# kthohr/mcmc

Measured on AMD Instinct MI355X. Metric: leapfrog-steps/sec (chains*dims*steps/s), HMC d=128 correlated Gaussian, 65536 chains, higher is better.
Workload: dtype f64

## Files before the change

include/mi_mcmc_engine/nuts_memo_core.hpp:

```cpp
#pragma once

#ifndef MI_MEMO_WALK_CAP
#define MI_MEMO_WALK_CAP 8
#endif

#ifndef MI_MEMO_RNG_ILP
#define MI_MEMO_RNG_ILP 1
#endif

#ifndef MI_MEMO_WALK_V2
#define MI_MEMO_WALK_V2 1
#endif
#ifndef MI_MEMO_APF
#define MI_MEMO_APF 0
#endif

#include "hmc_dense.hpp"

namespace mi {
namespace memo {

enum : int { NS_NEED_DRAW = 0, NS_TREE = 1, NS_DONE = 2,
             NS_INIT = 3, NS_SEARCH = 4,
             NS_WAIT = 5 };
enum : uint32_t { PQ_EMPTY = 0xffffffffu, PQ_GONE = 0xfffffffeu };
template <class T> __device__ __forceinline__ T coh_ld(const T* p) { return __hip_atomic_load(p, __ATOMIC_RELAXED, __HIP_MEMORY_SCOPE_AGENT); }
template <class T> __device__ __forceinline__ void coh_st(T* p, T v) { __hip_atomic_store(p, v, __ATOMIC_RELAXED, __HIP_MEMORY_SCOPE_AGENT); }
enum : int {
    MV_PREV = 0, MV_WPREV = 1, MV_MNTM = 2, MV_TPOS_T = 3, MV_TPOS_P = 4, MV_TNEG_T = 5, MV_TNEG_P = 6,
    MV_MNTM2 = 7, MV_PREVB = 8, MV_WPREVB = 9,
    MV_PT0 = 10,
    MEMO_MAXPTS = 46,
    MEMO_NVEC = MV_PT0 + 3 * MEMO_MAXPTS,
    MEMO_MAX_DEPTH = 10
};
enum : int {
    R_LA = 0,
    R_SC = 11,
    R_NF = 15,
    R_DA = 16,
    R_OKB = 19,
    R_LP = 31,
    R_CH = 42,
    R_CT = 49,
    R_END = 52
};
constexpr size_t lds_bytes() { return (size_t)R_END * 512 + 10 * 48 * 2; }

__host__ __device__ constexpr size_t memo_wave_bytes(int NS) { return (size_t)MEMO_NVEC * NS * 512 + (size_t)(MEMO_MAXPTS + 1) * 64 * 16; }

__device__ __forceinline__ uint32_t memo_npt(uint32_t i)
{
    return 1u + (uint32_t)__builtin_popcount(i) + (uint32_t)__builtin_popcount(i & 0x2AAu) + 2u * (uint32_t)__builtin_popcount(i & 0xCCu)
         + 4u * (uint32_t)__builtin_popcount(i & 0xF0u) + 8u * (uint32_t)__builtin_popcount(i & 0x300u);
}
__host__ __device__ inline bool memo_pair_used(int l, int n1, int j)
{
    const int m = n1 - 1;
    for (int t = 0; t <= j - l; ++t) {
        const int lo = t * (l + 1) + t * (t - 1) / 2, hi = t * j - t * (t - 1) / 2;
        if (m >= lo && m <= hi) return true;
    }
    return false;
}

template <int NT, class POL, class PRM>
__device__ __forceinline__ void nuts_memo_run(const PRM& prm, POL& pol, char* const lds_rows, uint16_t* const lds_pm)
{
    constexpr int NS = 4 * NT;
    for (int i = threadIdx.x; i < 10 * 48; i += blockDim.x) {
        const int j = i / 48, m = i % 48;
        uint32_t bits = 0;
        for (int l = 1; l <= j; ++l)
            if (m - l >= 1 && memo_pair_used(l, m - l, j)) bits |= 1u << l;
        lds_pm[i] = (uint16_t)bits;
    }
    __syncthreads();

    const int lane = threadIdx.x & 63, wave = threadIdx.x >> 6;
    const int j4 = lane >> 4;
    const int cw = wave * 16 + (lane & 15);
    const uint32_t d = prm.d;
    const uint64_t C = prm.C;
    const uint32_t nw = blockDim.x >> 6;
    const uint64_t n_slots = (uint64_t)gridDim.x * (16u * nw);
    uint64_t cl = ((uint64_t)blockIdx.x * nw + wave) * 16 + (lane & 15);
    bool exhausted = prm.next_chain == nullptr;
    uint32_t n_pieces = 1u, piece_len = 0xffffffffu;
    if constexpr (POL::SPLIT) { if (prm.n_pieces > 1u && prm.next_chain != nullptr) { n_pieces = prm.n_pieces; piece_len = prm.piece_len; } }
    const uint64_t n_items = C * (uint64_t)n_pieces;
    bool piece_done = false;

    typedef double __attribute__((address_space(3)))* lds_dptr;
    typedef unsigned long long __attribute__((address_space(3)))* lds_uptr;
    typedef char __attribute__((address_space(3)))* lds_bptr;
    uint32_t lrow = (uint32_t)(uintptr_t)(lds_bptr)lds_rows + (uint32_t)cw * 8u;
#define MI_RD(r) (*(lds_dptr)(uintptr_t)(lrow + (uint32_t)(r) * 512u))
#define MI_RU(r) (*(lds_uptr)(uintptr_t)(lrow + (uint32_t)(r) * 512u))
#define la_(l) MI_RD(R_LA + (l))
#define lp_(l) MI_RU(R_LP + (l))
#define okb_(r) MI_RU(R_OKB + (r))
#define nf_() MI_RD(R_NF)
    const int wave_u = __builtin_amdgcn_readfirstlane(wave);
    char* const ws_wave_u = reinterpret_cast<char*>(__builtin_assume_aligned(prm.ws, 256)) + ((size_t)blockIdx.x * nw + wave_u) * memo_wave_bytes(NS);
    uint32_t lane_b = (uint32_t)(lane & 15) * (uint32_t)(NS * 32) + (uint32_t)j4 * 16u;
    uint32_t lane_sc = (uint32_t)MEMO_NVEC * (uint32_t)(NS * 512) + (uint32_t)lane * 16u;
    auto wsp = [&](int v, int s) -> double* {
        return reinterpret_cast<double*>(ws_wave_u + ((uint32_t)v * (uint32_t)(NS * 512) + lane_b + (uint32_t)(s >> 1) * 64u));
    };
    auto scp = [&](uint32_t n) -> double2* { return reinterpret_cast<double2*>(ws_wave_u + (lane_sc + n * 1024u)); };
    auto ld_row = [&](int v, int s0, auto& dst) __attribute__((always_inline)) {
        constexpr int N = (int)(sizeof(dst) / sizeof(double));
        static_assert(N % 2 == 0, "rows move in pairs of slices");
#pragma unroll
        for (int k = 0; k < N; k += 2) {
            const double2 t = *reinterpret_cast<const double2*>(wsp(v, s0 + k));
            dst[k] = t.x; dst[k + 1] = t.y;
        }
    };
    auto st_row = [&](int v, int s0, const auto& src) __attribute__((always_inline)) {
        constexpr int N = (int)(sizeof(src) / sizeof(double));
        static_assert(N % 2 == 0, "rows move in pairs of slices");
#pragma unroll
        for (int k = 0; k < N; k += 2) *reinterpret_cast<double2*>(wsp(v, s0 + k)) = double2{src[k], src[k + 1]};
    };
#ifndef MI_MEMO_NT
#define MI_MEMO_NT 1
#endif
    [[maybe_unused]] auto st_row_nt = [&](int v, int s0, const auto& src) __attribute__((always_inline)) {
// ... 350 lines not shown
            if (gen) { next_K_() = kq / 2.0; next_lu_() = lu; mom_ready = true; }
            }
            const bool p = state == NS_NEED_DRAW;
            roll_state(p);
            if (max_depth > 0) begin_doubling(p);
            else { end_draw(p, 0u); if (p) state = NS_NEED_DRAW; }
        }
        const bool run = state == NS_TREE, init = state == NS_INIT, srch = state == NS_SEARCH;
        MI_MPROF(0)
        if (__ballot(run || init || srch) == 0ull) continue;
#ifdef MI_NUTS_REG_PROF
        n_ticks++; n_active += (unsigned long long)__builtin_popcountll(__ballot(run)) / 4ull;
        pc[10] += (unsigned long long)__builtin_popcountll(__ballot(run && memo_npt(li) > npts)) / 4ull;
#endif

        if (__ballot(init) != 0ull) {
#pragma unroll 1
            for (int b = 0; b < NS / 2; ++b) {
                const bool in0 = 8u * b + j4 < d, in1 = 8u * b + 4 + j4 < d;
                const double* src = prm.theta + ((size_t)(in0 ? 8u * b + j4 : 0u) * C + cl);
                double t0 = 0.0, t1 = 0.0;
                if (init) {
                    if constexpr (POL::SPLIT) { t0 = coh_ld(src); t1 = coh_ld(src + (in1 ? (size_t)4 * C : 0)); }
                    else { t0 = src[0]; t1 = src[in1 ? (size_t)4 * C : 0]; }
                }
                bool raw = false;
                if constexpr (POL::SPLIT) raw = draw != 0u;
                if (init) st_pair(MV_PREV, 2 * b, in0 ? (raw ? t0 : pol.enter(t0, 8 * b + j4)) : 0.0, in1 ? (raw ? t1 : pol.enter(t1, 8 * b + 4 + j4)) : 0.0);
            }
            const bool any_fresh = __ballot(init && prm.draw0 == 0 && draw == 0u) != 0ull;
#pragma unroll 1
            for (int b = 0; b < NS / 2; ++b) {
                double pa = 0.0, pb_ = 0.0;
                if (any_fresh) {
                    double z0, z1;
                    rng_normal_pair(prm.seed, prm.chain0 + cl, 0u, (uint32_t)(4 * b + j4), STREAM_INIT, z0, z1);
                    pa = (8u * b + j4 < d) ? z0 : 0.0;
                    pb_ = (8u * b + 4 + j4 < d) ? z1 : 0.0;
                    pa = pol.msqrt_times(pa, 8 * b + j4); pb_ = pol.msqrt_times(pb_, 8 * b + 4 + j4);
                }
                if (init) st_pair(mv, 2 * b, pa, pb_);
            }
        }
        const bool newpt = run && memo_npt(li) > npts;
        {
            const bool need = (newpt && npts == 0u && !org_ok) || init;
            if (__ballot(need) != 0ull) {
                const int vt = pvec(pb), vw = init ? pvec(pb) : wvec(pb);
                if (need) { ld_row(vt, 0, th); ld_draw_mom(init, pm); ld_row(vw, 0, w); }
            }
        }
        if (newpt) org_ok = false;
        const uint32_t mpt = npts + 1u;
        uint32_t pmask = newpt ? ((uint32_t)lds_pm[jd * 48u + mpt] | ((mpt == 1u + jd) ? 1u : 0u)) : 0u;
        auto test_vecs = [&](int l, int& vt, int& vp, bool& pmom) __attribute__((always_inline)) {
            vt = MV_PT0 + 3 * ((int)mpt - l - 1); vp = vt + 1; pmom = false;
            if (l == 0) {
                const bool oinit = (vdir > 0) ? neg_init : pos_init;
                vt = oinit ? pvec(pb0) : ((vdir > 0) ? MV_TNEG_T : MV_TPOS_T);
                vp = oinit ? mv : ((vdir > 0) ? MV_TNEG_P : MV_TPOS_P);
                pmom = oinit;
            }
        };
        auto ld_test_p = [&](int vp, bool pmom, auto& dst) __attribute__((always_inline)) {
            if constexpr (POL::PRE_MOM) ld_ptr(pmom ? mom_lane_ptr(draw) : ws_lane_ptr(vp), dst);
            else ld_row(vp, 0, dst);
        };
        double dd[NS], Lp[NS];
#pragma unroll
        for (int s_ = 0; s_ < NS; ++s_) { dd[s_] = 0.0; Lp[s_] = 0.0; }
        if (srch) {
            if (!s_first) eps_() = eps_() * ((vdir == 1) ? 2.0 : 0.5);
            n_leap_() += 1ull; n_exec_() += 1ull;
        }
        const double e_tick = newpt ? esg_() : (srch ? eps_() : 0.0);
#if MI_MEMO_APF > 0 && MI_MEMO_WALK_CAP > 0
        double apf[MI_MEMO_WALK_CAP];
#pragma unroll
        for (int k = 0; k < MI_MEMO_WALK_CAP; ++k) apf[k] = 0.0;
        auto request_alphas = [&]() __attribute__((always_inline)) {
            if (__ballot(run) == 0ull) return;
            uint32_t i_ = li, n_ = memo_npt(li);
            const uint32_t np_ = newpt ? mpt : npts;
            bool ok_ = run;
#pragma unroll
            for (int k = 0; k < MI_MEMO_WALK_CAP; ++k) {
                const uint32_t t_ = (uint32_t)__builtin_ctz(~i_);
                const uint32_t nn_ = n_ + (t_ + 1u) - t_ * (t_ + 1u) / 2u;
                ok_ = ok_ && nn_ <= np_;
                if (ok_ && !(newpt && nn_ == mpt)) apf[k] = scp(nn_)->x;
                i_ = i_ + 1u; n_ = nn_;
            }
        };
#endif
#if MI_MEMO_APF == 2 && MI_MEMO_WALK_CAP > 0
        request_alphas();
#endif
        const bool act = newpt || srch;
        pol.kick(th, pm, w, e_tick, act);
        pol.drift(th, pm, e_tick, act);
        __builtin_amdgcn_sched_barrier(0);
        {
            const bool t1 = pmask != 0u;
            if (__ballot(t1) != 0ull) {
                const int l1 = t1 ? __builtin_ctz(pmask) : 1;
                int vq, vqp; bool pmom;
                test_vecs(l1, vq, vqp, pmom);
                if (t1) { ld_row(vq, 0, dd); ld_test_p(vqp, pmom, Lp); }
            }
        }
        MI_MPROF(1)
        double val = 0.0;
        pol.eval(th, w, val);
        pol.kick(th, pm, w, e_tick, act);
        double pU = pol.potential(th, w, val);
        const double pK = pol.kinetic(pm);
        MI_MPROF(2)
        if (__ballot(init) != 0ull) {
            if (init) {
                st_row(MV_PREV, 0, th); st_row(MV_WPREV, 0, w);
                prev_U_() = pU;
                if constexpr (POL::REPLAY) { if (!is_finite(pU)) nf_() = 1.0; }
                H0_() = (is_finite(pU) ? pU : INF) + pK;
                s_first = true;
            }
            const bool cont = prm.draw0 != 0 || draw != 0u;
            if (init && cont) eps_() = prm.step_out ? coh_ld(prm.step_out + cl) : 1.0;
            start_sampling(init && cont);
            if (init && !cont) state = NS_SEARCH;
        }
        if (!is_finite(pU)) pU = INF;
        if (__ballot(srch) != 0ull) {
            const double dHs = -(pU + pK) + H0_();
            note_nonfinite(srch && !is_finite(dHs));
            if (srch) { vdir = 2 * (dHs > log_half ? 1 : 0) - 1; s_first = false; }
            start_sampling(srch && !(dHs > neg_log2));
        }
        MI_MPROF(5)
        if (__ballot(run) == 0ull) continue;
        const double dH = -(pU + pK) + H0_();
        note_nonfinite(newpt && !is_finite(dH));
        const double ca_pt = det_exp((dH < 0.0) ? dH : 0.0);
        if (newpt) {
            const unsigned long long bit = 1ull << mpt;
            const double lu_ = log_u_();
            const bool cn_b = lu_ <= -pU - pK;
            const bool cs_b = lu_ < 1000.0 - pU - pK;
            okb_(0) = (okb_(0) & ~bit) | (cn_b ? bit : 0ull);
            okb_(11) = (okb_(11) & ~bit) | (cs_b ? bit : 0ull);
            n_exec_() += 1ull;
        }
#if MI_MEMO_APF == 1 && MI_MEMO_WALK_CAP > 0
        request_alphas();
#endif
        MI_MPROF(8)
        {
            bool first = true;
#pragma unroll 1
            while (__ballot(pmask != 0u) != 0ull) {
#ifdef MI_NUTS_REG_PROF
                n_pair_it++;
#endif
                const bool t = pmask != 0u;
                const int l = t ? __builtin_ctz(pmask) : 1;
                const int n1 = (int)mpt - l;
                if (!first) {
                    int vq, vqp; bool pmom;
                    test_vecs(l, vq, vqp, pmom);
#if MI_MEMO_NT == 3
                    if (t) { ld_ptr_nt(ws_lane_ptr(vq), dd); if constexpr (POL::PRE_MOM) ld_ptr_nt(pmom ? mom_lane_ptr(draw) : ws_lane_ptr(vqp), Lp); else ld_ptr_nt(ws_lane_ptr(vqp), Lp); }
#else
                    if (t) { ld_row(vq, 0, dd); ld_test_p(vqp, pmom, Lp); }
#endif
                }
                first = false;
                double q1 = 0.0, q2 = 0.0;
#pragma unroll
                for (int s_ = 0; s_ < NS; ++s_) {
                    dd[s_] = (vdir > 0) ? (th[s_] - dd[s_]) : (dd[s_] - th[s_]);
                    q1 = dfma(dd[s_], Lp[s_], q1);
                }
                __builtin_amdgcn_sched_barrier(0);
#pragma unroll
                for (int s_ = 0; s_ < NS; ++s_) q2 = dfma(dd[s_], pm[s_], q2);
                q1 = q1 + __shfl_xor(q1, 32); q1 = q1 + __shfl_xor(q1, 16);
                q2 = q2 + __shfl_xor(q2, 32); q2 = q2 + __shfl_xor(q2, 16);
                if (t) {
                    const unsigned long long bit = (l == 0) ? (1ull << 63) : (1ull << n1);
                    const bool ok = (q1 >= 0.0) && (q2 >= 0.0);
                    okb_(l) = (okb_(l) & ~bit) | (ok ? bit : 0ull);
                    pmask &= pmask - 1u;
                }
            }
        }
        const bool st_edge = newpt && mpt == 1u + jd;
        if (st_edge) { if (vdir > 0) pos_init = false; else neg_init = false; }
        if (newpt) npts = mpt;
        MI_MPROF(3)
        bool wl = run;
        bool at_fin = false, complete = false;
        uint32_t cn_i = 0, cna_i = 0, cref = 0;
        double ca = newpt ? ca_pt : ca_keep;
        double ca_nx = 0.0;
        uint32_t n_walked = 0;
        uint32_t n = memo_npt(li);
#if MI_MEMO_WALK_CAP > 0
        int walk_budget = MI_MEMO_WALK_CAP;
#endif
#pragma unroll 1
        while (__ballot(wl) != 0ull) {
#ifdef MI_NUTS_REG_PROF
            n_walk_it++;
#endif
#if MI_MEMO_WALK_CAP > 0
            if (walk_budget-- == 0) break;
#endif
            const uint32_t t1 = (uint32_t)__builtin_ctz(~li);
            const uint32_t nn = n + (t1 + 1u) - t1 * (t1 + 1u) / 2u;
#if MI_MEMO_APF > 0 && MI_MEMO_WALK_CAP > 0
            ca_nx = (newpt && nn == mpt) ? ca_pt : apf[0];
#pragma unroll
            for (int k = 0; k + 1 < MI_MEMO_WALK_CAP; ++k) apf[k] = apf[k + 1];
#else
            if (wl && nn <= npts) ca_nx = (newpt && nn == mpt) ? ca_pt : scp(nn)->x;
#endif
            const unsigned long long nbit = 1ull << n;
            if (wl) {
                cn_i = (okb_(0) & nbit) ? 1u : 0u;
                cna_i = 1u; cref = n;
                n_walked++;
            }
            bool failed = wl && !(okb_(11) & nbit);
            uint32_t pend_level = jd + 1;
            if constexpr (MI_MEMO_WALK_V2 != 0 && POL::LANE_WALK) {
            const bool failed0 = failed;
            const uint32_t tm = wl ? t1 : 0u;
            uint32_t lb = 0;
#pragma unroll 1
            while (__ballot(lb < tm) != 0ull) {
                const bool act_r = lb < tm;
                const uint32_t cnt = act_r ? (((tm - lb) < 4u) ? (tm - lb) : 4u) : 0u;
                {
                    const bool stale = act_r && ((uslot - ub0) >= 4u || (uslot - ub0) + cnt > 4u);
                    if (__ballot(stale) != 0ull) {
// ... 104 lines not shown
            bool take = false;
            if (__ballot(complete) != 0ull) {
                const unsigned long long z = uni(complete);
                if (complete) {
                    uslot++;
                    take = u_below(z, cn_i, (uint32_t)n_val_());
                    if (take) { good_round = 1; pb = 1 - pb0; }
                }
            }
            const bool from_regs = take && newpt && cref == mpt;
            const bool from_rec = take && !from_regs;
            if (from_regs) { st_row(pvec(1 - pb0), 0, th); st_row(wvec(1 - pb0), 0, w); prev_U_() = pU; }
            if (__ballot(from_rec) != 0ull) {
                if (from_rec) prev_U_() = scp(cref)->y;
            }
            if (at_fin) { alpha_() = ca; n_alpha_() = (double)cna_i; n_val_() = n_val_() + (double)cn_i; }
            const bool s_ok = complete && ((okb_(0) >> 63) & 1ull) != 0ull;
            const bool more = at_fin && s_ok && (jd + 1 < max_depth);
            {
                const bool edge_now = st_edge && more;
                if (__ballot(edge_now) != 0ull) {
                    if (edge_now) { st_row((vdir > 0) ? MV_TPOS_T : MV_TNEG_T, 0, th); st_row((vdir > 0) ? MV_TPOS_P : MV_TNEG_P, 0, pm); }
                }
            }
            if (at_fin) jd = jd + 1;
            const bool ended = at_fin && !more;
            bool roll = false;
            if (__ballot(ended) != 0ull) {
                end_draw(ended, jd);
                roll = ended && draw < n_total && mom_ready && !row_pend && !piece_done;
                if (ended && !roll) state = NS_NEED_DRAW;
                roll_state(roll);
            }
            begin_doubling(more || roll);
            const bool go = more || roll;
            if (__ballot(go || from_rec) != 0ull) {
                if (from_rec) {
                    const int vq = MV_PT0 + 3 * ((int)cref - 1);
                    ld_row(vq, 0, th); ld_row(vq + 2, 0, w); cp_pend = true;
                }
                if (go) {
                    if (!take) { ld_row(pvec(pb), 0, th); ld_row(wvec(pb), 0, w); }
                    ld_draw_mom(false, pm);
                    org_ok = true;
                }
            }
        }
        MI_MPROF(9)
        {
            const bool rec = newpt && !at_fin;
            if (__ballot(rec) != 0ull) {
                if (rec) {
                    const int vr = MV_PT0 + 3 * ((int)mpt - 1);
#if MI_MEMO_NT == 1 || MI_MEMO_NT == 3
                    st_row(vr, 0, th); st_row(vr + 1, 0, pm); st_row_nt(vr + 2, 0, w);
#elif MI_MEMO_NT == 2
                    st_row_nt(vr, 0, th); st_row_nt(vr + 1, 0, pm); st_row_nt(vr + 2, 0, w);
#else
                    st_row(vr, 0, th); st_row(vr + 1, 0, pm); st_row(vr + 2, 0, w);
#endif
                    *scp(mpt) = double2{ca_pt, pU};
                    if (st_edge) {
                        st_row((vdir > 0) ? MV_TPOS_T : MV_TNEG_T, 0, th); st_row((vdir > 0) ? MV_TPOS_P : MV_TNEG_P, 0, pm);
                    }
                }
            }
        }
        MI_MPROF(6)
    }
#ifdef MI_NUTS_REG_PROF
    if (prm.prof && blockIdx.x == 0 && threadIdx.x == 0) {
        for (int k = 0; k < 12; ++k) prm.prof[k] = pc[k];
        prm.prof[12] = n_ticks; prm.prof[13] = n_active; prm.prof[14] = n_walk_it; prm.prof[15] = n_pair_it;
    }
#endif
#undef MI_MPROF
#undef la_
#undef lp_
#undef okb_
#undef nf_
#undef eps_
#undef prev_U_
#undef H0_
#undef log_u_
#undef esg_
#undef next_K_
#undef next_lu_
#undef n_leap_
#undef n_exec_
#undef n_acc_
#undef h_val_
#undef eps_bar_
#undef mu_val_
#undef prev_K_
#undef n_val_
#undef alpha_
#undef n_alpha_
#undef MI_RD
#undef MI_RU
}


}
}
```

include/mi_mcmc_engine/nuts_tile.hpp:

```cpp
#pragma once

#include "tile_samplers.hpp"
#include "nuts_memo_core.hpp"

namespace mi {

namespace tile_nuts {
enum : int { NUTS_MAX_DEPTH = memo::MEMO_MAX_DEPTH };
constexpr size_t lds_doubles() { return memo::lds_bytes() / sizeof(double); }
inline size_t ws_bytes(uint64_t n_chains, int nt) { return (size_t)((n_chains + 63) / 64) * 4 * memo::memo_wave_bytes(4 * nt); }
inline size_t ws_bytes_grid(uint64_t n_wg, int nt) { return (size_t)n_wg * 4 * memo::memo_wave_bytes(4 * nt); }

template <class T, bool GEN>
struct TileMemoPolicy {
    static constexpr int NT = T::NT, NS = 4 * NT;
    static constexpr bool REPLAY = false;
    static constexpr bool SPLIT = true;
    static constexpr bool PRE_MOM = false;
#ifndef MI_TILE_LANE_WALK
#define MI_TILE_LANE_WALK 1
#endif
    static constexpr bool LANE_WALK = MI_TILE_LANE_WALK != 0;
    const T& tgt;
    double* lds_t;
    const TileGen<T::NT>& tg;
    int j4;
    uint32_t d;
    __device__ __forceinline__ double enter(double v, int dim) const { if constexpr (GEN) return tg.enter(v, (uint32_t)dim); else return v; }
    __device__ __forceinline__ double leave(double v, int s) const { if constexpr (GEN) return tg.leave(v, s); else return v; }
    __device__ __forceinline__ double msqrt_times(double z, int dim) const { if constexpr (GEN) return tg.msqrt(dim) * z; else return z; }
    __device__ __forceinline__ double minv_times(double p, int dim) const { if constexpr (GEN) return tg.mi[dim] * p; else return 1.0 * p; }
    __device__ __forceinline__ void kick(const double (&th)[NS], double (&pm)[NS], const double (&w)[NS], double e, bool act) const
    {
        if constexpr (GEN) {
            double t[NS];
            tg.kick_terms(th, w, e, t);
#pragma unroll
            for (int s = 0; s < NS; ++s) pm[s] = act ? pm[s] + t[s] : pm[s];
        } else {
#pragma unroll
            for (int s = 0; s < NS; ++s) pm[s] = act ? pm[s] + (e * w[s]) / 2.0 : pm[s];
        }
    }
    __device__ __forceinline__ void drift(double (&th)[NS], const double (&pm)[NS], double e, bool act) const
    {
        if constexpr (GEN) {
            double mp[NS];
            tg.minv_p(pm, mp);
#pragma unroll
            for (int s = 0; s < NS; ++s) th[s] = act ? th[s] + e * mp[s] : th[s];
        } else {
            double t[NS];
#pragma unroll
            for (int s = 0; s < NS; ++s) t[s] = th[s] + e * pm[s];
            dense_product_poison<NS>(pm, t, j4, d);
#pragma unroll
            for (int s = 0; s < NS; ++s) th[s] = act ? t[s] : th[s];
        }
    }
    __device__ __forceinline__ void eval(const double (&th)[NS], double (&w)[NS], double& val) const
    {
        if constexpr (GEN) {
            double xs[NS];
            tg.x_of(th, xs);
            tgt.grad_tile(lds_t, xs, w, val, true);
        } else {
            tgt.grad_tile(lds_t, th, w, val, true);
        }
    }
    __device__ __forceinline__ double potential(const double (&th)[NS], const double (&)[NS], double val) const
    {
        if constexpr (GEN) return tg.potential(val, th);
        else return -val;
    }
    __device__ __forceinline__ double kinetic(const double (&p)[NS]) const
    {
        if constexpr (GEN) return tg.kinetic(p);
        else return diag_quadratic<NS>(p, 1.0, j4, d) / 2.0;
    }
};

template <class T, bool GEN = false>
__global__ MI_NO_DS_MERGE __launch_bounds__(256, 1) void nuts_tile_kernel(const TileParams prm, const T tgt)
{
    extern __shared__ __attribute__((aligned(16))) double lds_all[];
    double* const lds_t = lds_all;
    char* const lds_rows = reinterpret_cast<char*>(lds_all + prm.lds_user_doubles);
    uint16_t* const lds_pm = reinterpret_cast<uint16_t*>(lds_rows + memo::R_END * 512);
    [[maybe_unused]] double* const lds_gen = reinterpret_cast<double*>(lds_rows + memo::lds_bytes());
    tgt.stage(lds_t);
    if constexpr (GEN) TileGen<T::NT>::stage(lds_gen, prm);
    __syncthreads();
    TileGen<T::NT> tg;
    if constexpr (GEN) tg.use(lds_gen, prm);
    TileMemoPolicy<T, GEN> pol{tgt, lds_t, tg, (int)((threadIdx.x & 63) >> 4), prm.d};
    memo::nuts_memo_run<T::NT>(prm, pol, lds_rows, lds_pm);
}

}
using tile_nuts::nuts_tile_kernel;

}
```

mcmc_amd/__init__.py:

```python
import ctypes as C
import os

import numpy as np

_HERE = os.path.dirname(os.path.abspath(__file__))
LIB_PATH = os.path.join(_HERE, "libmi_mcmc.so")

MI_OK, MI_ERR_BAD_ARG, MI_ERR_HIP, MI_ERR_UNSUPPORTED, MI_ERR_OOM, MI_ERR_NO_DEVICE = range(6)
TARGET_GAUSS_ISO, TARGET_GAUSS_DIAG, TARGET_GAUSS_DENSE, TARGET_LOGISTIC, TARGET_NORMAL_MODEL = 1, 2, 3, 4, 5
TARGET_GAUSS_MIXTURE = 6
MEM_HOST, MEM_DEVICE = 0, 1
KERNEL_AUTO, KERNEL_ELEMENTWISE_1LANE, KERNEL_ELEMENTWISE_4LANE, KERNEL_NUTS_LOCKSTEP = 0, 1, 2, 3
KERNEL_HMC_TWO_WAVES_PER_SIMD, KERNEL_HMC_ONE_WAVE_PER_SIMD, KERNEL_HMC_SPLIT2, KERNEL_HMC_SPLIT4, KERNEL_HMC_SPLIT4_TWO_WAVES = 4, 5, 6, 7, 8
KERNEL_NUTS_TICK_LOCAL, KERNEL_NUTS_REG, KERNEL_NUTS_SPLIT, KERNEL_LITERAL, KERNEL_NUTS_DYN, KERNEL_NUTS_MEMO, KERNEL_NUTS_MEMO_INTICK = 9, 10, 11, 12, 13, 14, 15

_dp = C.POINTER(C.c_double)
_u64p = C.POINTER(C.c_uint64)


class mi_target(C.Structure):
    _fields_ = [("struct_size", C.c_uint32), ("kind", C.c_int32), ("d", C.c_uint64),
                ("prec", C.c_void_p), ("X", C.c_void_p), ("y", C.c_void_p),
                ("n_rows", C.c_uint64), ("mem", C.c_int32), ("kernel_hint", C.c_int32)]

# ... 10 lines not shown


class mi_chains(C.Structure):
    _fields_ = [("struct_size", C.c_uint32), ("mem", C.c_int32), ("n_chains", C.c_uint64),
                ("chain0", C.c_uint64), ("theta", C.c_void_p), ("draws", C.c_void_p),
                ("n_accept", C.c_void_p), ("step_size", C.c_void_p), ("n_leapfrogs", C.c_void_p),
                ("nuts_depth", C.c_void_p), ("draw0", C.c_uint64), ("nuts_adapt_state", C.c_void_p), ("mass_diag", C.c_void_p),
                ("n_leapfrogs_executed", C.c_void_p)]


class mi_de_settings(C.Structure):
    _fields_ = [("struct_size", C.c_uint32), ("jumps", C.c_int32), ("n_pop", C.c_uint64), ("par_b", C.c_double),
                ("par_gamma_jump", C.c_double), ("par_gamma", C.c_double), ("initial_lb", C.c_void_p), ("initial_ub", C.c_void_p)]


class mi_populations(C.Structure):
    _fields_ = [("struct_size", C.c_uint32), ("mem", C.c_int32), ("n_populations", C.c_uint64), ("population0", C.c_uint64),
                ("initial_vals", C.c_void_p), ("population", C.c_void_p), ("draws", C.c_void_p), ("n_accept", C.c_void_p),
                ("draw0", C.c_uint64)]


class mi_aees_settings(C.Structure):
    _fields_ = [("struct_size", C.c_uint32), ("n_rings", C.c_uint32), ("n_initial_draws", C.c_uint64), ("par_scale", C.c_double),
                ("cov_mat", C.c_void_p), ("ee_prob_par", C.c_double), ("temper_vec", C.c_void_p), ("temper_len", C.c_uint64)]


class mi_aees_runs(C.Structure):
    _fields_ = [("struct_size", C.c_uint32), ("mem", C.c_int32), ("n_runs", C.c_uint64), ("run0", C.c_uint64),
                ("initial_vals", C.c_void_p), ("draws", C.c_void_p), ("final_states", C.c_void_p), ("n_accept", C.c_void_p),
                ("n_ee_accept", C.c_void_p)]


class MiMcmcError(RuntimeError):
    def __init__(self, code, msg):
        super().__init__(f"mi_mcmc status {code}: {msg}")
        self.code = code


_lib = None

EXPORTS = [
    "mi_settings_default", "mi_mcmc_last_error", "mi_mcmc_last_kernel", "mi_mcmc_version", "mi_mcmc_device_count", "mi_mcmc_release_workspace", "mi_mcmc_run_user_target", "mi_mcmc_run_user_target_v", "mi_mcmc_run_tile_target",
    "mi_mcmc_hmc_run", "mi_mcmc_mala_run", "mi_mcmc_nuts_run", "mi_mcmc_rwmh_run", "mi_mcmc_rmhmc_run", "mi_mcmc_hmc_run_mass_adapted", "mi_mcmc_hmc_run_mass_adapted_per_chain", "mi_mcmc_hmc_run_callback", "mi_mcmc_mala_run_callback", "mi_mcmc_nuts_run_callback", "mi_mcmc_rwmh_run_callback", "mi_mcmc_rmhmc_run_callback",
    "mi_de_settings_default", "mi_mcmc_de_run", "mi_mcmc_de_run_callback",
    "mi_aees_settings_default", "mi_mcmc_aees_run", "mi_mcmc_aees_run_callback",
    "mi_mcmc_draws_to_chain_major", "mi_mcmc_draws_to_chain_major_device", "mi_mcmc_shard_bounds", "mi_mcmc_allgather_draws", "mi_mcmc_allgather_draws_ragged", "mi_mcmc_merge_shards", "mi_mcmc_draw_stats",
    "mi_mcmc_allgather_draws_rank_major", "mi_mcmc_rank_major_index", "mi_mcmc_allgather_draws_begin", "mi_mcmc_allgather_draws_wait",
    "mi_mcmc_mat_inverse", "mi_mcmc_mat_cholesky_lower",
    "mi_mcmc_draws_covariance", "mi_mcmc_hmc_run_mass_adapted_dense", "mi_mcmc_mala_run_mass_adapted_dense",
    "mi_mcmc_draws_order_stats", "mi_mcmc_draws_quantiles",
    "mi_mcmc_draws_rank_transform", "mi_mcmc_draw_stats_ranked", "mi_mcmc_norm_ppf",
    "mi_mcmc_draws_log_kernel",
]
PROBE_EXPORTS = ["mi_probe_mfma_f64", "mi_probe_math", "mi_probe_normals", "mi_probe_uniform", "mi_probe_fp64_peak", "mi_probe_mfma_cycles"]


def _one_hip_runtime():
    import importlib.util
    import sys
    if "torch" in sys.modules:
        return
    try:
        spec = importlib.util.find_spec("torch")
    except (ImportError, ValueError):
        spec = None
    if spec is None or not spec.origin:
        return
    libdir = os.path.join(os.path.dirname(spec.origin), "lib")
    for name in ("libhsa-runtime64.so", "libamdhip64.so"):
        p = os.path.join(libdir, name)
        if os.path.exists(p):
            try:
                C.CDLL(p, mode=C.RTLD_GLOBAL)
            except OSError:
                pass


def lib():
    global _lib
    if _lib is None:
        path = os.environ.get("MI_MCMC_LIB", LIB_PATH)
        if not os.path.exists(path):
            raise MiMcmcError(-1, f"{path} not built: run `make -C mcmc_amd/csrc` (no CPU fallback)")
        _one_hip_runtime()
        _lib = C.CDLL(path)
        _lib.mi_mcmc_last_error.restype = C.c_char_p
        _lib.mi_mcmc_last_kernel.restype = C.c_char_p
    return _lib


_plib = None


def probes_lib():
    global _plib
    if _plib is None:
        lib()
        path = os.path.join(os.path.dirname(LIB_PATH), "libmi_mcmc_probes.so")
        if not os.path.exists(path):
            raise MiMcmcError(-1, f"{path} not built: run `make -C mcmc_amd/csrc`")
        _plib = C.CDLL(path)
    return _plib


def _check(rc):
    if rc != MI_OK:
        raise MiMcmcError(rc, lib().mi_mcmc_last_error().decode())
# ... 415 lines not shown
        cb = LOG_KERNEL_CB(_tramp)
    else:
        cb = callback
    _check(lib().mi_mcmc_aees_run_callback(C.c_void_p(x0.ctypes.data), C.c_uint64(d), C.cast(cb, C.c_void_p), C.c_void_p(target_data or 0),
                                           C.byref(settings), C.byref(a), C.c_void_p(draws.ctypes.data), C.c_void_p(fin.ctypes.data),
                                           C.c_void_p(n_acc.ctypes.data), C.c_void_p(n_ee.ctypes.data)))
    return draws, dict(final_states=fin, n_accept=n_acc, n_ee_accept=n_ee)


def probe_mfma(A, B, Cin):
    A = np.ascontiguousarray(A, dtype=np.float64)
    B = np.ascontiguousarray(B, dtype=np.float64)
    Cin = np.ascontiguousarray(Cin, dtype=np.float64)
    D = np.zeros((16, 16))
    _check(probes_lib().mi_probe_mfma_f64(C.c_void_p(A.ctypes.data), C.c_void_p(B.ctypes.data),
                                   C.c_void_p(Cin.ctypes.data), C.c_void_p(D.ctypes.data)))
    return D


def probe_math(fn, x):
    x = np.ascontiguousarray(x, dtype=np.float64)
    o1, o2 = np.empty_like(x), np.empty_like(x)
    _check(probes_lib().mi_probe_math(fn, C.c_void_p(x.ctypes.data), C.c_uint64(x.size),
                               C.c_void_p(o1.ctypes.data), C.c_void_p(o2.ctypes.data)))
    return o1, o2


def probe_normals(seed, chain, draw, stream, d):
    out = np.zeros(d)
    _check(probes_lib().mi_probe_normals(C.c_uint64(seed), C.c_uint64(chain), C.c_uint32(draw),
                                  C.c_uint32(stream), C.c_uint64(d), C.c_void_p(out.ctypes.data)))
    return out


def probe_uniform(seed, chain, draw, slot):
    out = np.zeros(1)
    _check(probes_lib().mi_probe_uniform(C.c_uint64(seed), C.c_uint64(chain), C.c_uint32(draw),
                                  C.c_uint32(slot), C.c_void_p(out.ctypes.data)))
    return float(out[0])


def probe_fp64_peak(use_mfma, iters=20000):
    out = C.c_double(0.0)
    _check(probes_lib().mi_probe_fp64_peak(int(use_mfma), int(iters), C.byref(out)))
    return out.value


def probe_mfma_cycles(waves_per_simd, use_lds, iters=20000):
    cyc, tf = C.c_double(0.0), C.c_double(0.0)
    _check(probes_lib().mi_probe_mfma_cycles(int(waves_per_simd), int(use_lds), int(iters), C.byref(cyc), C.byref(tf)))
    return cyc.value, tf.value


def mat_inverse(A):
    A = np.ascontiguousarray(A, dtype=np.float64)
    d = A.shape[0]
    out = np.empty((d, d))
    _check(lib().mi_mcmc_mat_inverse(C.c_void_p(A.ctypes.data), C.c_uint64(d), C.c_void_p(out.ctypes.data)))
    return out


def mat_cholesky_lower(A):
    A = np.ascontiguousarray(A, dtype=np.float64)
    d = A.shape[0]
    out = np.empty((d, d))
    _check(lib().mi_mcmc_mat_cholesky_lower(C.c_void_p(A.ctypes.data), C.c_uint64(d), C.c_void_p(out.ctypes.data)))
    return out


def draw_stats(draws, n_keep=None, d=None, n_chains=None, mem=MEM_HOST, stream=None, want_acov=True):
    if mem == MEM_HOST:
        draws = np.ascontiguousarray(draws, dtype=np.float64)
        n_keep, d, n_chains = draws.shape
    mean = np.zeros(d)
    acov = np.zeros((n_keep, d)) if want_acov else None
    rhat, ess = np.zeros(d), np.zeros(d)
    _check(lib().mi_mcmc_draw_stats(C.c_void_p(_ptr(draws)), C.c_int32(mem), C.c_uint64(n_keep), C.c_uint64(d), C.c_uint64(n_chains),
                                    C.c_void_p(mean.ctypes.data), C.c_void_p(acov.ctypes.data if want_acov else 0), C.c_void_p(rhat.ctypes.data),
                                    C.c_void_p(ess.ctypes.data), C.c_void_p(stream or 0)))
    return dict(mean=mean, acov=acov, rhat=rhat, ess=ess)


def test_draw_stats_last():
    o = (C.c_uint64 * 8)()
    lib().mi_mcmc_test_draw_stats_last(o)
    return dict(zip(("route", "NB", "G", "tiles", "window_launches", "lag_passes", "subset_passes", "smallest_subset"), (int(v) for v in o)))


def draws_covariance(draws, n_keep=None, d=None, n_chains=None, mem=MEM_HOST, stream=None, want_mean=True, want_cov=True):
    if mem == MEM_HOST:
        draws = np.ascontiguousarray(draws, dtype=np.float64)
        if draws.ndim == 2:
            draws = draws[None]
        n_keep, d, n_chains = draws.shape
    mean = np.zeros(d) if want_mean else None
    cov = np.zeros((d, d)) if want_cov else None
    _check(lib().mi_mcmc_draws_covariance(C.c_void_p(_ptr(draws)), C.c_int32(mem), C.c_uint64(n_keep), C.c_uint64(d), C.c_uint64(n_chains),
                                          C.c_void_p(_ptr(mean)), C.c_void_p(_ptr(cov)), C.c_void_p(stream or 0)))
    return mean, cov


def _slab_shape(draws, n_keep, d, n_chains, mem):
    if mem == MEM_HOST:
        draws = np.ascontiguousarray(draws, dtype=np.float64)
        if draws.ndim == 2:
            draws = draws[None]
# ... 86 lines not shown
```

mcmc_amd/csrc/mi_mcmc_probes.h:

```cpp
#pragma once
#include <stdint.h>
#ifdef __cplusplus
extern "C" {
#endif
int mi_probe_mfma_f64(const double* A16x4, const double* B4x16, const double* C16x16, double* D16x16);
int mi_probe_math(int fn, const double* x, uint64_t n, double* out, double* out2);
int mi_probe_normals(uint64_t seed, uint64_t chain, uint32_t draw, uint32_t stream, uint64_t d, double* out);
int mi_probe_uniform(uint64_t seed, uint64_t chain, uint32_t draw, uint32_t slot, double* out);
int mi_probe_fp64_peak(int use_mfma, int iters, double* tflops_out);
int mi_probe_mfma_cycles(int waves_per_simd, int use_lds, int iters, double* cycles_per_mfma, double* tflops_out);
void mi_mcmc_test_set_grid_cap(uint32_t max_workgroups);
void mi_mcmc_test_set_linalg_stage_bytes(uint32_t bytes);
uint64_t mi_mcmc_test_linalg_computed(void);
uint64_t mi_mcmc_test_linalg_computed_on_device(void);
void mi_mcmc_test_set_gemm_nuts_ws_bytes(uint64_t bytes);
uint64_t mi_mcmc_test_gemm_nuts_ranges(void);
void mi_mcmc_test_gemm_nuts_last_ticks(uint64_t* ticks, uint64_t* busy_slots, uint64_t* slots);
uint64_t mi_mcmc_test_gemm_nuts_tick_ceiling(uint32_t max_tree_depth, uint64_t n_draws, int search);
uint64_t mi_mcmc_test_gemm_nuts_chain_bytes(uint32_t d, uint32_t n_rows, uint32_t max_tree_depth);
uint64_t mi_mcmc_test_gemm_nuts_fixed_bytes(uint32_t d, uint32_t n_rows);
uint64_t mi_mcmc_test_gemm_nuts_range_chains(uint64_t n_chains, uint64_t chain_bytes, uint64_t fixed_bytes, uint64_t budget);
void mi_mcmc_test_set_gemm_graph(int mode);
void mi_mcmc_test_set_gemm_ws_bytes(uint64_t bytes);
uint64_t mi_mcmc_test_gemm_need_bytes(uint32_t d, uint32_t n_rows, uint64_t n_chains, int variant, int replay);
void mi_mcmc_test_set_rank_ws_bytes(uint64_t bytes);
uint64_t mi_mcmc_test_rank_dim_bytes(uint64_t n_keep, uint64_t n_chains, uint32_t flags, int stats);
uint64_t mi_mcmc_test_rank_dims_per_group(uint64_t n_keep, uint64_t d, uint64_t n_chains, uint32_t flags, int stats);
void mi_mcmc_test_rank_counts(uint64_t* sorts, uint64_t* passes);
void mi_mcmc_test_logk_plan(int32_t kind, uint64_t d, uint64_t n_rows, uint64_t n_keep, uint64_t n_chains, int slab_host, int target_host, uint64_t* out8);
void mi_mcmc_test_draw_stats_last(uint64_t* out8);
#ifdef __cplusplus
}
#endif
```

mcmc_amd/csrc/nuts_memo.hpp:

```cpp

#pragma once

#include "nuts_async.hpp"
#include "nuts_memo_core.hpp"

namespace mi {

using memo::memo_wave_bytes;

template <int NT, bool DIAGM, bool PRE = false>
struct GaussMemoPolicy {
    static constexpr int NS = 4 * NT;
    static constexpr bool REPLAY = true;
    static constexpr bool PRE_MOM = PRE;
    static constexpr bool SPLIT = true;
    static constexpr bool LANE_WALK = !(DIAGM && NT == 8);
    const double* afrag;
    const double* lds_ms;
    const double* lds_mi;
    __device__ __forceinline__ const double* mcol(const double* tab) const
    {
        const double* p = tab + ((threadIdx.x & 63) >> 4);
        asm volatile("" : "+v"(p));
        return p;
    }
    __device__ __forceinline__ double enter(double v, int) const { return v; }
    __device__ __forceinline__ double leave(double v, int) const { return v; }
    __device__ __forceinline__ double msqrt_times(double z, int dim) const { if constexpr (DIAGM) return lds_ms[dim] * z; else return z; }
    __device__ __forceinline__ double minv_times(double p, int dim) const { if constexpr (DIAGM) return lds_mi[dim] * p; else return p; }
    __device__ __forceinline__ void kick(const double (&)[NS], double (&pm)[NS], const double (&w)[NS], double e, bool) const
    {
#pragma unroll
        for (int s = 0; s < NS; ++s) pm[s] = pm[s] - (e * w[s]) / 2.0;
    }
    __device__ __forceinline__ void drift(double (&th)[NS], const double (&pm)[NS], double e, bool) const
    {
        if constexpr (DIAGM) {
            const double* mic = mcol(lds_mi);
#pragma unroll
            for (int s = 0; s < NS; ++s) th[s] = th[s] + e * (mic[4 * s] * pm[s]);
        } else {
#pragma unroll
            for (int s = 0; s < NS; ++s) th[s] = th[s] + e * pm[s];
        }
    }
    __device__ __forceinline__ void eval(const double (&th)[NS], double (&w)[NS], double&) const { matvec_mfma<NT>(afrag, th, w); }
    __device__ __forceinline__ double potential(const double (&th)[NS], const double (&w)[NS], double) const { return 0.5 * dot4<NS>(th, w); }
    __device__ __forceinline__ double kinetic(const double (&p)[NS]) const
    {
        if constexpr (DIAGM) {
            const double* mic = mcol(lds_mi);
            double q = 0.0;
#pragma unroll
            for (int s = 0; s < NS; ++s) q = dfma(p[s], mic[4 * s] * p[s], q);
            q = q + __shfl_xor(q, 32);
            q = q + __shfl_xor(q, 16);
            return q / 2.0;
        } else {
            return dot4<NS>(p, p) / 2.0;
        }
    }
};

template <int NT, bool DIAGM>
__global__ __launch_bounds__(256) void nuts_momenta_kernel(const NutsParams prm)
{
    constexpr int NS = 4 * NT;
    const int lane = threadIdx.x & 63, j4 = lane >> 4;
    const uint32_t d = prm.d;
    const uint64_t n_tiles = (prm.C + 15) / 16;
    const uint64_t wid = (uint64_t)blockIdx.x * 4 + (threadIdx.x >> 6);
    const uint32_t n_total = prm.n_burnin + prm.n_keep;
    if (wid >= n_tiles * (uint64_t)n_total) return;
    const uint32_t k = (uint32_t)(wid / n_tiles);
    const uint64_t c = (wid % n_tiles) * 16 + (uint64_t)(lane & 15);
    const bool live = c < prm.C;
    const uint64_t cc = live ? c : prm.C - 1;
    char* const base = reinterpret_cast<char*>(prm.mom) + (((size_t)k * prm.C + cc) * (size_t)(NS * 32) + (size_t)j4 * 16u);
    double kq = 0.0;
#pragma unroll 2
    for (int b = 0; b < NS / 2; ++b) {
        double z0, z1;
        rng_normal_pair(prm.seed, prm.chain0 + cc, k + prm.draw0, (uint32_t)(4 * b + j4), STREAM_NORMAL, z0, z1);
        const uint32_t da = 8u * b + j4, db = 8u * b + 4u + j4;
        double pa = (da < d) ? z0 : 0.0;
        double pb_ = (db < d) ? z1 : 0.0;
        if constexpr (DIAGM) {
            const double msa = (da < d) ? prm.m_sqrt[da] : 1.0, msb = (db < d) ? prm.m_sqrt[db] : 1.0;
            const double mia = (da < d) ? prm.m_inv[da] : 1.0, mib = (db < d) ? prm.m_inv[db] : 1.0;
            pa = msa * pa; pb_ = msb * pb_;
            kq = dfma(pa, mia * pa, kq);
            kq = dfma(pb_, mib * pb_, kq);
        } else {
            kq = dfma(pa, pa, kq);
            kq = dfma(pb_, pb_, kq);
        }
// ... 36 lines not shown
```

mcmc_amd/csrc/probes.hip:

```cpp
#include <hip/hip_runtime.h>

#include <cstring>

#include "host_common.hpp"
#include "mi_mcmc_probes.h"
#include "det_math.hpp"
#include "hmc_dense.hpp"

using mi::host::fail;
using mi::host::DevBuf;

namespace {

__global__ void probe_mfma_kernel(const double* A, const double* B, const double* Cin, double* D)
{
    const int l = threadIdx.x;
    const double a = A[(l & 15) * 4 + (l >> 4)];
    const double b = B[(l >> 4) * 16 + (l & 15)];
    mi::double4_t c;
    for (int r = 0; r < 4; ++r) c[r] = Cin[((l >> 4) + 4 * r) * 16 + (l & 15)];
    c = __builtin_amdgcn_mfma_f64_16x16x4f64(a, b, c, 0, 0, 0);
    for (int r = 0; r < 4; ++r) D[((l >> 4) + 4 * r) * 16 + (l & 15)] = c[r];
}

__global__ void probe_math_kernel(int fn, const double* x, uint64_t n, double* out, double* out2)
{
    const uint64_t i = (uint64_t)blockIdx.x * blockDim.x + threadIdx.x;
    if (i >= n) return;
    double s = 0.0, c = 0.0;
    switch (fn) {
    case 0: s = mi::det_exp(x[i]); break;
    case 1: s = mi::det_log(x[i]); break;
    case 2: mi::det_sincos2pi(x[i], s, c); break;
    case 3: s = mi::softplus(x[i]); break;
    case 4: s = mi::sigmoid(x[i]); break;
    default: s = __builtin_nan("");
    }
    out[i] = s;
    out2[i] = c;
}

__global__ void probe_normals_kernel(uint64_t seed, uint64_t chain, uint32_t draw, uint32_t stream, uint64_t d, double* out)
{
    const uint64_t slot = (uint64_t)blockIdx.x * blockDim.x + threadIdx.x;
    const uint64_t nslots = 4 * ((d + 7) / 8);
    if (slot >= nslots) return;
    const uint64_t b = slot / 4, j = slot % 4;
    const uint64_t i0 = 8 * b + j, i1 = i0 + 4;
    double z0, z1;
    mi::rng_normal_pair(seed, chain, draw, (uint32_t)slot, stream, z0, z1);
    if (i0 < d) out[i0] = z0;
    if (i1 < d) out[i1] = z1;
}

__global__ void probe_uniform_kernel(uint64_t seed, uint64_t chain, uint32_t draw, uint32_t slot, double* out)
{
    out[0] = mi::rng_uniform(seed, chain, draw, slot);
}

__global__ __launch_bounds__(256) void peak_mfma_kernel(int iters, double* sink)
// ... 109 lines not shown
    DevBuf sink, cyc;
    HIP_TRY(sink.alloc(8)); HIP_TRY(cyc.alloc(8));
    hipEvent_t e0, e1;
    HIP_TRY(hipEventCreate(&e0)); HIP_TRY(hipEventCreate(&e1));
    const int grid = 256 * waves_per_simd;
    const int nacc_req = (use_lds >> 8) & 0xff;
    const int nacc = (nacc_req == 1 || nacc_req == 2 || nacc_req == 4) ? nacc_req : 8;
    for (int rep = 0; rep < 2; ++rep) {
        HIP_TRY(hipEventRecord(e0, 0));
        if (nacc == 1) hipLaunchKernelGGL((mfma_cycles_kernel<1, false>), dim3(grid), dim3(256), 0, 0, iters, cyc.as<unsigned long long>(), sink.as<double>());
        else if (nacc == 2) hipLaunchKernelGGL((mfma_cycles_kernel<2, false>), dim3(grid), dim3(256), 0, 0, iters, cyc.as<unsigned long long>(), sink.as<double>());
        else if (nacc == 4) hipLaunchKernelGGL((mfma_cycles_kernel<4, false>), dim3(grid), dim3(256), 0, 0, iters, cyc.as<unsigned long long>(), sink.as<double>());
        else if (use_lds & 1) hipLaunchKernelGGL((mfma_cycles_kernel<8, true>), dim3(grid), dim3(256), 0, 0, iters, cyc.as<unsigned long long>(), sink.as<double>());
        else hipLaunchKernelGGL((mfma_cycles_kernel<8, false>), dim3(grid), dim3(256), 0, 0, iters, cyc.as<unsigned long long>(), sink.as<double>());
        HIP_TRY(hipEventRecord(e1, 0));
        HIP_TRY(hipEventSynchronize(e1));
    }
    float ms = 0.f;
    HIP_TRY(hipEventElapsedTime(&ms, e0, e1));
    unsigned long long c = 0;
    HIP_TRY(hipMemcpy(&c, cyc.p, 8, hipMemcpyDeviceToHost));
    *cycles_per_mfma = (double)c / ((double)iters * nacc);
    *tflops_out = (double)grid * 4 * iters * (double)nacc * 2048.0 / (ms * 1e-3) / 1e12;
    (void)hipEventDestroy(e0); (void)hipEventDestroy(e1);
    return MI_OK;
}

int mi_probe_fp64_peak(int use_mfma, int iters, double* tflops_out)
{
    if (!tflops_out || iters <= 0) return fail(MI_ERR_BAD_ARG, "bad args");
    DevBuf sink;
    HIP_TRY(sink.alloc(8));
    hipEvent_t e0, e1;
    HIP_TRY(hipEventCreate(&e0));
    HIP_TRY(hipEventCreate(&e1));
    const int grid = 256 * 8;
    for (int rep = 0; rep < 2; ++rep) {
        HIP_TRY(hipEventRecord(e0, 0));
        if (use_mfma) hipLaunchKernelGGL(peak_mfma_kernel, dim3(grid), dim3(256), 0, 0, iters, sink.as<double>());
        else hipLaunchKernelGGL(peak_fma_kernel, dim3(grid), dim3(256), 0, 0, iters, sink.as<double>());
        HIP_TRY(hipEventRecord(e1, 0));
        HIP_TRY(hipEventSynchronize(e1));
    }
    float ms = 0.f;
    HIP_TRY(hipEventElapsedTime(&ms, e0, e1));
    const double waves = (double)grid * 4;
    const double flop = use_mfma ? waves * iters * 8.0 * (16.0 * 16 * 4 * 2) : waves * iters * 16.0 * 64 * 2;
    *tflops_out = flop / (ms * 1e-3) / 1e12;
    (void)hipEventDestroy(e0);
    (void)hipEventDestroy(e1);
    return MI_OK;
}

}
```

Measured before the change: 265.9 billion.

## Keep level-1 NUTS memo test vectors in registers instead of reloading rows

During the leapfrog step the previous theta and momentum are captured in registers (kick_keep/drift_keep), so the level-1 U-turn pair test uses them directly instead of loading stored rows from memory. A new bit in the precomputed pair-usage table marks points whose momentum is ever read at level two or higher, and storing the momentum row is skipped when it is not needed. This trades extra register pressure and extra copies for fewer memory loads and stores per tree point. A probe export for the table is also added.

```diff
diff --git a/include/mi_mcmc_engine/nuts_memo_core.hpp b/include/mi_mcmc_engine/nuts_memo_core.hpp
--- a/include/mi_mcmc_engine/nuts_memo_core.hpp
+++ b/include/mi_mcmc_engine/nuts_memo_core.hpp
@@ -13,6 +13,9 @@
 #endif
 #ifndef MI_MEMO_APF
 #define MI_MEMO_APF 0
+#endif
+#ifndef MI_MEMO_L1REG
+#define MI_MEMO_L1REG 1
 #endif
 
 #include "hmc_dense.hpp"
@@ -63,18 +66,22 @@
     }
     return false;
 }
+__host__ __device__ inline uint32_t memo_pm_entry(int j, int m)
+{
+    uint32_t bits = 0;
+    for (int l = 1; l <= j; ++l)
+        if (m - l >= 1 && memo_pair_used(l, m - l, j)) bits |= 1u << l;
+    for (int l = 2; l <= j; ++l)
+        if (m >= 1 && memo_pair_used(l, m, j)) bits |= 1u << 15;
+    return bits;
+}
 
 template <int NT, class POL, class PRM>
 __device__ __forceinline__ void nuts_memo_run(const PRM& prm, POL& pol, char* const lds_rows, uint16_t* const lds_pm)
 {
     constexpr int NS = 4 * NT;
-    for (int i = threadIdx.x; i < 10 * 48; i += blockDim.x) {
-        const int j = i / 48, m = i % 48;
-        uint32_t bits = 0;
-        for (int l = 1; l <= j; ++l)
-            if (m - l >= 1 && memo_pair_used(l, m - l, j)) bits |= 1u << l;
-        lds_pm[i] = (uint16_t)bits;
-    }
+    for (int i = threadIdx.x; i < 10 * 48; i += blockDim.x)
+        lds_pm[i] = (uint16_t)(memo_pm_entry(i / 48, i % 48) & (MI_MEMO_L1REG != 0 ? 0xffffu : 0x7fffu));
     __syncthreads();
 
     const int lane = threadIdx.x & 63, wave = threadIdx.x >> 6;
@@ -531,7 +538,10 @@
         }
         if (newpt) org_ok = false;
         const uint32_t mpt = npts + 1u;
-        uint32_t pmask = newpt ? ((uint32_t)lds_pm[jd * 48u + mpt] | ((mpt == 1u + jd) ? 1u : 0u)) : 0u;
+        constexpr uint32_t PM_LEVELS = MI_MEMO_L1REG != 0 ? 0x7fffu : 0xffffu;
+        uint32_t pmask = newpt ? (((uint32_t)lds_pm[jd * 48u + mpt] & PM_LEVELS) | ((mpt == 1u + jd) ? 1u : 0u)) : 0u;
+        constexpr bool L1R = MI_MEMO_L1REG != 0 && POL::L1_REGS;
+        auto next_level = [](uint32_t pmk) __attribute__((always_inline)) -> int { return (L1R && (pmk & 2u) != 0u) ? 1 : __builtin_ctz(pmk); };
         auto test_vecs = [&](int l, int& vt, int& vp, bool& pmom) __attribute__((always_inline)) {
             vt = MV_PT0 + 3 * ((int)mpt - l - 1); vp = vt + 1; pmom = false;
             if (l == 0) {
@@ -576,16 +586,22 @@
         request_alphas();
 #endif
         const bool act = newpt || srch;
-        pol.kick(th, pm, w, e_tick, act);
-        pol.drift(th, pm, e_tick, act);
+        if constexpr (L1R) {
+            pol.kick_keep(th, pm, w, e_tick, act, Lp);
+            pol.drift_keep(th, pm, e_tick, act, dd);
+        } else {
+            pol.kick(th, pm, w, e_tick, act);
+            pol.drift(th, pm, e_tick, act);
+        }
         __builtin_amdgcn_sched_barrier(0);
         {
             const bool t1 = pmask != 0u;
-            if (__ballot(t1) != 0ull) {
-                const int l1 = t1 ? __builtin_ctz(pmask) : 1;
+            const int l1 = t1 ? next_level(pmask) : 1;
+            const bool ld1 = t1 && !(L1R && l1 == 1);
+            if (__ballot(ld1) != 0ull) {
                 int vq, vqp; bool pmom;
                 test_vecs(l1, vq, vqp, pmom);
-                if (t1) { ld_row(vq, 0, dd); ld_test_p(vqp, pmom, Lp); }
+                if (ld1) { ld_row(vq, 0, dd); ld_test_p(vqp, pmom, Lp); }
             }
         }
         MI_MPROF(1)
@@ -641,7 +657,7 @@
                 n_pair_it++;
 #endif
                 const bool t = pmask != 0u;
-                const int l = t ? __builtin_ctz(pmask) : 1;
+                const int l = t ? next_level(pmask) : 1;
                 const int n1 = (int)mpt - l;
                 if (!first) {
                     int vq, vqp; bool pmom;
@@ -668,7 +684,7 @@
                     const unsigned long long bit = (l == 0) ? (1ull << 63) : (1ull << n1);
                     const bool ok = (q1 >= 0.0) && (q2 >= 0.0);
                     okb_(l) = (okb_(l) & ~bit) | (ok ? bit : 0ull);
-                    pmask &= pmask - 1u;
+                    pmask &= L1R ? ~(1u << l) : (pmask - 1u);
                 }
             }
         }
@@ -879,12 +895,14 @@
             if (__ballot(rec) != 0ull) {
                 if (rec) {
                     const int vr = MV_PT0 + 3 * ((int)mpt - 1);
+                    bool keep_p = true;
+                    if constexpr (L1R) keep_p = (((uint32_t)lds_pm[jd * 48u + mpt] >> 15) & 1u) != 0u;
 #if MI_MEMO_NT == 1 || MI_MEMO_NT == 3
-                    st_row(vr, 0, th); st_row(vr + 1, 0, pm); st_row_nt(vr + 2, 0, w);
+                    st_row(vr, 0, th); if (keep_p) st_row(vr + 1, 0, pm); st_row_nt(vr + 2, 0, w);
 #elif MI_MEMO_NT == 2
-                    st_row_nt(vr, 0, th); st_row_nt(vr + 1, 0, pm); st_row_nt(vr + 2, 0, w);
+                    st_row_nt(vr, 0, th); if (keep_p) st_row_nt(vr + 1, 0, pm); st_row_nt(vr + 2, 0, w);
 #else
-                    st_row(vr, 0, th); st_row(vr + 1, 0, pm); st_row(vr + 2, 0, w);
+                    st_row(vr, 0, th); if (keep_p) st_row(vr + 1, 0, pm); st_row(vr + 2, 0, w);
 #endif
                     *scp(mpt) = double2{ca_pt, pU};
                     if (st_edge) {
diff --git a/include/mi_mcmc_engine/nuts_tile.hpp b/include/mi_mcmc_engine/nuts_tile.hpp
--- a/include/mi_mcmc_engine/nuts_tile.hpp
+++ b/include/mi_mcmc_engine/nuts_tile.hpp
@@ -21,6 +21,7 @@
 #define MI_TILE_LANE_WALK 1
 #endif
     static constexpr bool LANE_WALK = MI_TILE_LANE_WALK != 0;
+    static constexpr bool L1_REGS = true;
     const T& tgt;
     double* lds_t;
     const TileGen<T::NT>& tg;
@@ -56,6 +57,34 @@
             dense_product_poison<NS>(pm, t, j4, d);
 #pragma unroll
             for (int s = 0; s < NS; ++s) th[s] = act ? t[s] : th[s];
+        }
+    }
+    __device__ __forceinline__ void kick_keep(const double (&th)[NS], double (&pm)[NS], const double (&w)[NS], double e, bool act, double (&old)[NS]) const
+    {
+        if constexpr (GEN) {
+            double t[NS];
+            tg.kick_terms(th, w, e, t);
+#pragma unroll
+            for (int s = 0; s < NS; ++s) { old[s] = pm[s]; pm[s] = act ? pm[s] + t[s] : pm[s]; asm volatile("" : "+v"(pm[s])); }
+        } else {
+#pragma unroll
+            for (int s = 0; s < NS; ++s) { old[s] = pm[s]; pm[s] = act ? pm[s] + (e * w[s]) / 2.0 : pm[s]; asm volatile("" : "+v"(pm[s])); }
+        }
+    }
+    __device__ __forceinline__ void drift_keep(double (&th)[NS], const double (&pm)[NS], double e, bool act, double (&old)[NS]) const
+    {
+        if constexpr (GEN) {
+            double mp[NS];
+            tg.minv_p(pm, mp);
+#pragma unroll
+            for (int s = 0; s < NS; ++s) { old[s] = th[s]; th[s] = act ? th[s] + e * mp[s] : th[s]; }
+        } else {
+            double t[NS];
+#pragma unroll
+            for (int s = 0; s < NS; ++s) t[s] = th[s] + e * pm[s];
+            dense_product_poison<NS>(pm, t, j4, d);
+#pragma unroll
+            for (int s = 0; s < NS; ++s) { old[s] = th[s]; th[s] = act ? t[s] : th[s]; }
         }
     }
     __device__ __forceinline__ void eval(const double (&th)[NS], double (&w)[NS], double& val) const
diff --git a/mcmc_amd/__init__.py b/mcmc_amd/__init__.py
--- a/mcmc_amd/__init__.py
+++ b/mcmc_amd/__init__.py
@@ -86,7 +86,7 @@
     "mi_mcmc_draws_rank_transform", "mi_mcmc_draw_stats_ranked", "mi_mcmc_norm_ppf",
     "mi_mcmc_draws_log_kernel",
 ]
-PROBE_EXPORTS = ["mi_probe_mfma_f64", "mi_probe_math", "mi_probe_normals", "mi_probe_uniform", "mi_probe_fp64_peak", "mi_probe_mfma_cycles"]
+PROBE_EXPORTS = ["mi_probe_mfma_f64", "mi_probe_math", "mi_probe_normals", "mi_probe_uniform", "mi_probe_fp64_peak", "mi_probe_mfma_cycles", "mi_probe_nuts_memo_table"]
 
 
 def _one_hip_runtime():
@@ -608,6 +608,12 @@
     return cyc.value, tf.value
 
 
+def probe_nuts_memo_table():
+    out = np.zeros((10, 48), dtype=np.uint16)
+    _check(probes_lib().mi_probe_nuts_memo_table(C.c_void_p(out.ctypes.data)))
+    return out
+
+
 def mat_inverse(A):
     A = np.ascontiguousarray(A, dtype=np.float64)
     d = A.shape[0]
diff --git a/mcmc_amd/csrc/mi_mcmc_probes.h b/mcmc_amd/csrc/mi_mcmc_probes.h
--- a/mcmc_amd/csrc/mi_mcmc_probes.h
+++ b/mcmc_amd/csrc/mi_mcmc_probes.h
@@ -9,6 +9,7 @@
 int mi_probe_uniform(uint64_t seed, uint64_t chain, uint32_t draw, uint32_t slot, double* out);
 int mi_probe_fp64_peak(int use_mfma, int iters, double* tflops_out);
 int mi_probe_mfma_cycles(int waves_per_simd, int use_lds, int iters, double* cycles_per_mfma, double* tflops_out);
+int mi_probe_nuts_memo_table(uint16_t* out480);
 void mi_mcmc_test_set_grid_cap(uint32_t max_workgroups);
 void mi_mcmc_test_set_linalg_stage_bytes(uint32_t bytes);
 uint64_t mi_mcmc_test_linalg_computed(void);
diff --git a/mcmc_amd/csrc/nuts_memo.hpp b/mcmc_amd/csrc/nuts_memo.hpp
--- a/mcmc_amd/csrc/nuts_memo.hpp
+++ b/mcmc_amd/csrc/nuts_memo.hpp
@@ -15,6 +15,7 @@
     static constexpr bool PRE_MOM = PRE;
     static constexpr bool SPLIT = true;
     static constexpr bool LANE_WALK = !(DIAGM && NT == 8);
+    static constexpr bool L1_REGS = true;
     const double* afrag;
     const double* lds_ms;
     const double* lds_mi;
@@ -42,6 +43,26 @@
         } else {
 #pragma unroll
             for (int s = 0; s < NS; ++s) th[s] = th[s] + e * pm[s];
+        }
+    }
+    __device__ __forceinline__ void kick_keep(const double (&)[NS], double (&pm)[NS], const double (&w)[NS], double e, bool, double (&old)[NS]) const
+    {
+#pragma unroll
+        for (int s = 0; s < NS; ++s) {
+            old[s] = pm[s];
+            pm[s] = pm[s] - (e * w[s]) / 2.0;
+            asm volatile("" : "+v"(pm[s]));
+        }
+    }
+    __device__ __forceinline__ void drift_keep(double (&th)[NS], const double (&pm)[NS], double e, bool, double (&old)[NS]) const
+    {
+        if constexpr (DIAGM) {
+            const double* mic = mcol(lds_mi);
+#pragma unroll
+            for (int s = 0; s < NS; ++s) { old[s] = th[s]; th[s] = th[s] + e * (mic[4 * s] * pm[s]); }
+        } else {
+#pragma unroll
+            for (int s = 0; s < NS; ++s) { old[s] = th[s]; th[s] = th[s] + e * pm[s]; }
         }
     }
     __device__ __forceinline__ void eval(const double (&th)[NS], double (&w)[NS], double&) const { matvec_mfma<NT>(afrag, th, w); }
diff --git a/mcmc_amd/csrc/probes.hip b/mcmc_amd/csrc/probes.hip
--- a/mcmc_amd/csrc/probes.hip
+++ b/mcmc_amd/csrc/probes.hip
@@ -6,6 +6,7 @@
 #include "mi_mcmc_probes.h"
 #include "det_math.hpp"
 #include "hmc_dense.hpp"
+#include "nuts_memo_core.hpp"
 
 using mi::host::fail;
 using mi::host::DevBuf;
@@ -221,4 +222,11 @@
     return MI_OK;
 }
 
-}
+int mi_probe_nuts_memo_table(uint16_t* out480)
+{
+    if (!out480) return fail(MI_ERR_BAD_ARG, "bad args");
+    for (int i = 0; i < 10 * 48; ++i) out480[i] = (uint16_t)mi::memo::memo_pm_entry(i / 48, i % 48);
+    return MI_OK;
+}
+
+}
```

New measurement: 265.7 billion. About the same (-0.1%).
